# yuxiaoxiangyong/Multilateral-Temporal-view-Pyramid-Transformer-for-Video-Inpainting-Detection

Measured on AMD Instinct MI355X. Metric: clips/sec fwd (B=8,T=5,224x224), higher is better.
Workload: dtype f32; 1 GPU; full Mumpy forward (3 temporal views, pyramid decoder), B=8 clips/GPU, T=5, 224x224, fp32, tubelets (5,4,1); global_batch=8, launch=hipGraph replay, fork/join over HIP streams (independent branches co-scheduled), parallelism=batch-sharded x1, one metric all-reduce

## Files before the change

### multilateral-temporal-view-pyramid-transformer-for-video-inpainting-detection_amd/csrc/abi.cpp

```cpp
#include <stdarg.h>
#include <stdio.h>
#include <string.h>
#include "common.h"
#include "../../include/mumpy_hip_ext.h"
#include "../../include/mumpy_hip_ext2.h"
#include "../../include/mumpy_hip_ext3.h"
#include "../../include/mumpy_hip_ext4.h"
#include "../../include/mumpy_hip_ext5.h"
#include "../../include/mumpy_hip_ext6.h"
#include "../../include/mumpy_hip_ext7.h"
#include "../../include/mumpy_hip_ext8.h"
#include "../../include/mumpy_hip_ext9.h"
#include "../../include/mumpy_hip_ext10.h"
#include "../../include/mumpy_perturb.h"

namespace mumpy {
static thread_local char g_err[512] = "";
void set_error(const char* fmt, ...) {
    va_list ap;
    va_start(ap, fmt);
    vsnprintf(g_err, sizeof(g_err), fmt, ap);
    va_end(ap);
}
thread_local Route g_route;
static thread_local char g_route_text[160] = "";
static const char* format_route() {
    static const char* const addr[] = {"dense", "rows", "kseg", "conv"};
    static const char* const ln[] = {"none", "producer", "consumer"};
    static const char* const red[] = {"none", "one", "two-in-one", "taps"};
    const Route& r = g_route;
    char* t = g_route_text;
    const size_t n = sizeof(g_route_text);
    switch (r.family) {
    case Route::TILED: snprintf(t, n, "tiled tile=%d ks=%d np=%d addr=%s", r.tile, r.ks, r.np, addr[r.addr & 3]); break;
    case Route::TILED16: snprintf(t, n, "tiled16 tile=%d ks=%d np=%d addr=%s", r.tile, r.ks, r.np, addr[r.addr & 3]); break;
    case Route::WS:
        snprintf(t, n, "ws sched=%s P=%d ln=%s addr=%s", r.split ? "split" : "whole", r.passes, ln[r.ln < 3 ? r.ln : 0], addr[r.addr & 3]);
        break;
    case Route::WS64: snprintf(t, n, "ws64 P=%d addr=dense", r.passes); break;
    case Route::WS16: snprintf(t, n, "ws16 P=%d addr=dense", r.passes); break;
    case Route::XGEMM: {
        char dx[24] = "-", dw[24] = "-";
        if (r.prod[0].wt) snprintf(dx, sizeof(dx), "%dx%d", r.prod[0].wt, r.prod[0].ks);
        if (r.prod[1].wt) snprintf(dw, sizeof(dw), "%dx%d", r.prod[1].wt, r.prod[1].ks);
        snprintf(t, n, "xgemm np=%d addr=%s dx=%s dw=%s reduce=%s", r.np, addr[r.addr & 3], dx, dw, red[r.reduce & 3]);
        break;
    }
    default: snprintf(t, n, "none");
    }
    if (r.dual && r.family != Route::NONE) {
        const size_t len = strlen(t);
        snprintf(t + len, n - len, r.family == Route::XGEMM ? " gate=gelu" : " dual=z");
    }
    return t;
}
#ifdef MUMPY_TUNING
#include <stdlib.h>
int tune_int(const char* name, int dflt) {
    const char* v = getenv(name);
    return v ? atoi(v) : dflt;
}
const char* tune_str(const char* name) { return getenv(name); }
#endif
}

extern "C" int mumpy_tuning_build(void) {
#ifdef MUMPY_TUNING
    return 1;
#else
    return 0;
#endif
}

extern "C" int mumpy_abi_version(void) { return MUMPY_ABI_VERSION; }
extern "C" int mumpy_ext_version(void) { return MUMPY_EXT_VERSION; }
extern "C" int mumpy_ext2_version(void) { return MUMPY_EXT2_VERSION; }
extern "C" int mumpy_ext3_version(void) { return MUMPY_EXT3_VERSION; }
extern "C" int mumpy_ext4_version(void) { return MUMPY_EXT4_VERSION; }
extern "C" int mumpy_ext5_version(void) { return MUMPY_EXT5_VERSION; }
extern "C" int mumpy_ext6_version(void) { return MUMPY_EXT6_VERSION; }
extern "C" int mumpy_ext7_version(void) { return MUMPY_EXT7_VERSION; }
extern "C" int mumpy_ext8_version(void) { return MUMPY_EXT8_VERSION; }
extern "C" int mumpy_ext9_version(void) { return MUMPY_EXT9_VERSION; }
extern "C" int mumpy_ext10_version(void) { return MUMPY_EXT10_VERSION; }
extern "C" int mumpy_perturb_version(void) { return MUMPY_PERTURB_VERSION; }
extern "C" const char* mumpy_last_error(void) { return mumpy::g_err; }
extern "C" const char* mumpy_last_route(void) { return mumpy::format_route(); }
```

### multilateral-temporal-view-pyramid-transformer-for-video-inpainting-detection_amd/csrc/cva_fused.hip

```cpp
#include "cva_pairing.h"
#include "../../include/mumpy_hip_ext8.h"
using namespace mumpy;

namespace {

constexpr int BK = 32, LDR = 36;
constexpr int LDH = 20;

typedef __bf16 bf16x8 __attribute__((ext_vector_type(8)));
typedef __bf16 bf16x4 __attribute__((ext_vector_type(4)));

__device__ __forceinline__ void put_bf16x4(float* img, int dw, f32x4 v) {
    *reinterpret_cast<uint2*>(img + dw) = __builtin_bit_cast(uint2, __builtin_convertvector(v, bf16x4));
}
__device__ __forceinline__ bf16x8 frag_bf16(const float* row_h, int st) { return *reinterpret_cast<const bf16x8*>(row_h + 8 * st); }

__device__ __forceinline__ void divmod49(unsigned m, unsigned& q, unsigned& r) {
    q = (unsigned)(((uint64_t)m * 2804876602ull) >> 37);
    r = m - 49u * q;
}

template <int C, bool MM16, bool GROUPED>
__global__ __launch_bounds__(256, 2) void deform_sample_kv_kernel(const float* __restrict__ x2, const float* __restrict__ pos,
                                                                  const float* __restrict__ Wkv, const float* __restrict__ bkv,
                                                                  float* __restrict__ kv, int Hs2, int W, int nWx, int nW2,
                                                                  CvaPairing<GROUPED> pair, int M, unsigned gn) {
    constexpr int BM = 64, BN = 192, TN = 3, N = 2 * C, K = C, CG = C / 3, NK = K / BK, CPG = CG / BK;
    constexpr int A_LD = BM / 32, B_LD = BN / 32;
    __shared__ __attribute__((aligned(16))) float lds[2][(BM + BN) * (MM16 ? LDH : LDR)];
    const int tid = threadIdx.x, lane = tid & 63, wave = tid >> 6;
    const int c = lane & 31, h = lane >> 5, wm = wave >> 1, wn = wave & 1;
    const unsigned wgid = xcd_major_id(blockIdx.x, gridDim.x);
    const unsigned tm = wgid / gn, tn = wgid - tm * gn;
    const int m0 = (int)tm * BM, n0 = (int)tn * BN;
    const int ld_row = tid >> 3, ld_c4 = tid & 7;

    const float* abase[A_LD];
    const float* apos[A_LD];
    int aoff[A_LD][4];
    float aw[A_LD][4];
#pragma unroll
    for (int i = 0; i < A_LD; ++i) {
        int m = m0 + ld_row + 32 * i;
        if (m > M - 1) m = M - 1;
        unsigned b2, p;
        divmod49((unsigned)m, b2, p);
        const unsigned b = b2 / (unsigned)nW2, n = b2 - b * (unsigned)nW2;
        const unsigned wy = n / (unsigned)nWx, wx = n - wy * (unsigned)nWx;
        abase[i] = x2 + (((int64_t)b * Hs2 + wy * WS) * W + wx * WS) * C + 4 * ld_c4;
        apos[i] = pos + ((int64_t)cva_q_window(b2, pair) * 3 * WT + p) * 2;
    }
    auto set_group = [&](int g) {
#pragma unroll
        for (int i = 0; i < A_LD; ++i) {
            const float gy = apos[i][g * WT * 2], gx = apos[i][g * WT * 2 + 1];
            const float iy = ((gy + 1.0f) * 0.5f) * 6.0f;
            const float ix = ((gx + 1.0f) * 0.5f) * 6.0f;
            const float y0f = floorf(iy), x0f = floorf(ix);
            const int y0 = (int)y0f, x0 = (int)x0f;
            const float wgt[4] = {(x0f + 1.0f - ix) * (y0f + 1.0f - iy), (ix - x0f) * (y0f + 1.0f - iy),
                                  (x0f + 1.0f - ix) * (iy - y0f), (ix - x0f) * (iy - y0f)};
#pragma unroll
            for (int e = 0; e < 4; ++e) {
                const int yy = y0 + (e >> 1), xx = x0 + (e & 1);
                const bool ok = (unsigned)yy < (unsigned)WS && (unsigned)xx < (unsigned)WS;
                aw[i][e] = ok ? wgt[e] : 0.f;
                aoff[i][e] = ok ? (yy * W + xx) * C : 0;
            }
        }
    };
    const float* brow[B_LD];
#pragma unroll
    for (int i = 0; i < B_LD; ++i) {
        int n = n0 + ld_row + 32 * i;
        if (n > N - 1) n = N - 1;
        brow[i] = Wkv + (int64_t)n * K + 4 * ld_c4;
    }
    f32x4 areg[A_LD], breg[B_LD];
    auto gload = [&](int kc) {
        const int k0 = kc * BK;
#pragma unroll
        for (int i = 0; i < A_LD; ++i) {
            const float* s = abase[i] + k0;
            f32x4 r = *reinterpret_cast<const f32x4*>(s + aoff[i][0]) * aw[i][0];
            r += *reinterpret_cast<const f32x4*>(s + aoff[i][1]) * aw[i][1];
            r += *reinterpret_cast<const f32x4*>(s + aoff[i][2]) * aw[i][2];
            r += *reinterpret_cast<const f32x4*>(s + aoff[i][3]) * aw[i][3];
            areg[i] = r;
        }
#pragma unroll
        for (int i = 0; i < B_LD; ++i) breg[i] = *reinterpret_cast<const f32x4*>(brow[i] + k0);
    };
    auto lstore = [&](int buf) {
        if constexpr (MM16) {
#pragma unroll
            for (int i = 0; i < A_LD; ++i) put_bf16x4(lds[buf], (ld_row + 32 * i) * LDH + 2 * ld_c4, areg[i]);
#pragma unroll
            for (int i = 0; i < B_LD; ++i) put_bf16x4(lds[buf], (BM + ld_row + 32 * i) * LDH + 2 * ld_c4, breg[i]);
        } else {
#pragma unroll
            for (int i = 0; i < A_LD; ++i) *reinterpret_cast<f32x4*>(&lds[buf][(ld_row + 32 * i) * LDR + 4 * ld_c4]) = areg[i];
#pragma unroll
            for (int i = 0; i < B_LD; ++i) *reinterpret_cast<f32x4*>(&lds[buf][(BM + ld_row + 32 * i) * LDR + 4 * ld_c4]) = breg[i];
        }
    };
    f32x16 acc[TN];
#pragma unroll
    for (int j = 0; j < TN; ++j)
#pragma unroll
        for (int r = 0; r < 16; ++r) acc[j][r] = 0.f;
    auto compute = [&](int buf) {
        if constexpr (MM16) {
            const float* a_f = &lds[buf][(wm * 32 + c) * LDH + 4 * h];
            const float* b_f = &lds[buf][(BM + wn * 96 + c) * LDH + 4 * h];
#pragma unroll
            for (int st = 0; st < 2; ++st) {
                const bf16x8 fa = frag_bf16(a_f, st);
                bf16x8 fb[TN];
#pragma unroll
                for (int j = 0; j < TN; ++j) fb[j] = frag_bf16(b_f + 32 * j * LDH, st);
#pragma unroll
                for (int j = 0; j < TN; ++j) acc[j] = __builtin_amdgcn_mfma_f32_32x32x16_bf16(fa, fb[j], acc[j], 0, 0, 0);
            }
        } else {
            const float* a_f = &lds[buf][(wm * 32 + c) * LDR + 16 * h];
            const float* b_f = &lds[buf][(BM + wn * 96 + c) * LDR + 16 * h];
#pragma unroll
            for (int q = 0; q < 4; ++q) {
                const f32x4 fa = *reinterpret_cast<const f32x4*>(a_f + 4 * q);
                f32x4 fb[TN];
#pragma unroll
                for (int j = 0; j < TN; ++j) fb[j] = *reinterpret_cast<const f32x4*>(b_f + 32 * j * LDR + 4 * q);
#pragma unroll
                for (int e = 0; e < 4; ++e)
#pragma unroll
                    for (int j = 0; j < TN; ++j) acc[j] = __builtin_amdgcn_mfma_f32_32x32x2f32(fa[e], fb[j][e], acc[j], 0, 0, 0);
            }
        }
    };
    set_group(0);
    gload(0);
    lstore(0);
    __syncthreads();
    for (int kc = 0; kc < NK; ++kc) {
        if (kc + 1 < NK) {
            if ((kc + 1) % CPG == 0) set_group((kc + 1) / CPG);
            gload(kc + 1);
        }
        compute(kc & 1);
        if (kc + 1 < NK) lstore((kc + 1) & 1);
        __syncthreads();
    }
#pragma unroll
    for (int j = 0; j < TN; ++j) {
        const int n = n0 + wn * 96 + 32 * j + c;
        if (n >= N) continue;
        const float bv = bkv[n];
#pragma unroll
        for (int r = 0; r < 16; ++r) {
            const int m = m0 + wm * 32 + (r & 3) + 8 * (r >> 2) + 4 * h;
            if (m < M) kv[(int64_t)m * N + n] = acc[j][r] + bv;
        }
    }
}

template <int C, bool MM16>
__global__ __launch_bounds__(256, 2) void deform_out_combine_kernel(const float* __restrict__ o, const float* __restrict__ Wout,
                                                                   const float* __restrict__ bout, const float* __restrict__ x1,
                                                                   float* __restrict__ out, int H, int W, int nWx, int nWf, int MO,
                                                                   unsigned gn) {
    constexpr int BM = 64, BN = 64, K = C, NK = K / BK;
    constexpr int A_LD = BM / 32, B_LD = BN / 32;
    __shared__ __attribute__((aligned(16))) float lds[2][(BM + BN) * (MM16 ? LDH : LDR)];
    const int tid = threadIdx.x, lane = tid & 63, wave = tid >> 6;
    const int c = lane & 31, h = lane >> 5, wm = wave >> 1, wn = wave & 1;
    const unsigned wgid = xcd_major_id(blockIdx.x, gridDim.x);
    const unsigned tn = wgid / gn, tm = wgid - tn * gn;
    const int c0 = (int)tm * BM, m0 = (int)tn * BN;
    const int ld_row = tid >> 3, ld_c4 = tid & 7;
    const float* arow[A_LD];
    const float* brow[B_LD];
#pragma unroll
    for (int i = 0; i < A_LD; ++i) {
        int cc = c0 + ld_row + 32 * i;
        if (cc > C - 1) cc = C - 1;
        arow[i] = Wout + (int64_t)cc * K + 4 * ld_c4;
    }
#pragma unroll
    for (int i = 0; i < B_LD; ++i) {
        int m = m0 + ld_row + 32 * i;
        if (m > MO - 1) m = MO - 1;
        brow[i] = o + (int64_t)m * K + 4 * ld_c4;
    }
    f32x4 areg[A_LD], breg[B_LD];
    auto gload = [&](int kc) {
#pragma unroll
        for (int i = 0; i < A_LD; ++i) areg[i] = *reinterpret_cast<const f32x4*>(arow[i] + kc * BK);
#pragma unroll
        for (int i = 0; i < B_LD; ++i) breg[i] = *reinterpret_cast<const f32x4*>(brow[i] + kc * BK);
    };
    auto lstore = [&](int buf) {
        if constexpr (MM16) {
#pragma unroll
            for (int i = 0; i < A_LD; ++i) put_bf16x4(lds[buf], (ld_row + 32 * i) * LDH + 2 * ld_c4, areg[i]);
#pragma unroll
            for (int i = 0; i < B_LD; ++i) put_bf16x4(lds[buf], (BM + ld_row + 32 * i) * LDH + 2 * ld_c4, breg[i]);
        } else {
#pragma unroll
            for (int i = 0; i < A_LD; ++i) *reinterpret_cast<f32x4*>(&lds[buf][(ld_row + 32 * i) * LDR + 4 * ld_c4]) = areg[i];
#pragma unroll
            for (int i = 0; i < B_LD; ++i) *reinterpret_cast<f32x4*>(&lds[buf][(BM + ld_row + 32 * i) * LDR + 4 * ld_c4]) = breg[i];
        }
    };
    f32x16 acc;
#pragma unroll
    for (int r = 0; r < 16; ++r) acc[r] = 0.f;
    auto compute = [&](int buf) {
        if constexpr (MM16) {
            const float* a_f = &lds[buf][(wm * 32 + c) * LDH + 4 * h];
            const float* b_f = &lds[buf][(BM + wn * 32 + c) * LDH + 4 * h];
#pragma unroll
            for (int st = 0; st < 2; ++st)
                acc = __builtin_amdgcn_mfma_f32_32x32x16_bf16(frag_bf16(a_f, st), frag_bf16(b_f, st), acc, 0, 0, 0);
        } else {
            const float* a_f = &lds[buf][(wm * 32 + c) * LDR + 16 * h];
            const float* b_f = &lds[buf][(BM + wn * 32 + c) * LDR + 16 * h];
#pragma unroll
            for (int q = 0; q < 4; ++q) {
                const f32x4 fa = *reinterpret_cast<const f32x4*>(a_f + 4 * q), fb = *reinterpret_cast<const f32x4*>(b_f + 4 * q);
#pragma unroll
                for (int e = 0; e < 4; ++e) acc = __builtin_amdgcn_mfma_f32_32x32x2f32(fa[e], fb[e], acc, 0, 0, 0);
            }
        }
    };
    gload(0);
    lstore(0);
    __syncthreads();
    for (int kc = 0; kc < NK; ++kc) {
        if (kc + 1 < NK) gload(kc + 1);
        compute(kc & 1);
        if (kc + 1 < NK) lstore((kc + 1) & 1);
        __syncthreads();
    }
    const int m = m0 + wn * 32 + c;
    if (m >= MO) return;
    unsigned bw, pp;
    divmod49((unsigned)m, bw, pp);
    const unsigned b = bw / (unsigned)nWf, n = bw - b * (unsigned)nWf;
    const int wy = (int)(n / (unsigned)nWx), wx = (int)(n - (n / (unsigned)nWx) * (unsigned)nWx);
    const int64_t img = (int64_t)b * H * W;
    const int64_t win_base = (img + (int64_t)n * WT) * C;
#pragma unroll
    for (int r = 0; r < 16; ++r) {
        const int cc = c0 + wm * 32 + (r & 3) + 8 * (r >> 2) + 4 * h;
        if (cc >= C) continue;
        const int f = cc * WT + (int)pp;
        const int po = f / C, co = f - po * C;
        const int tok = window_token(wy, wx, po, H, W, 0);
        out[win_base + f] = x1[win_base + f] + x1[(img + tok) * C + co] + (acc[r] + bout[cc]);
    }
}

}

template <bool MM16>
static int sample_kv_launch(const char* who, const float* x2, const float* pos, const float* Wkv, const float* bkv, float* kv, int B,
                            int Hs2, int W, int C, int nq, int groups, void* stream) {
    MUMPY_REQUIRE(x2 && pos && Wkv && bkv && kv, MUMPY_ENULL, "%s: null pointer", who);
    MUMPY_REQUIRE(aligned16(x2) && aligned16(Wkv) && aligned16(kv), MUMPY_EALIGN, "%s: pointers must be 16-byte aligned", who);
    MUMPY_REQUIRE(B > 0 && Hs2 > 0 && W > 0 && Hs2 % WS == 0 && W % WS == 0 && nq > 0, MUMPY_EINVAL,
                  "%s: bad grid (%d,%d) / nq=%d", who, Hs2, W, nq);
    MUMPY_REQUIRE(C == 96 || C == 192 || C == 384 || C == 768, MUMPY_EINVAL,
                  "%s: C=%d is not one of the encoder widths 96/192/384/768", who, C);
    const int nWx = W / WS, nW2 = (Hs2 / WS) * nWx;
    const int64_t nwin = (int64_t)B * nW2, M = nwin * WT;
    MUMPY_REQUIRE(M < (1ll << 31) - 64, MUMPY_ERANGE, "%s: too many windows", who);
    const unsigned gn = (unsigned)((2 * C + 191) / 192);
    const int64_t grid = ((M + 63) / 64) * gn;
    MUMPY_REQUIRE(grid < (1ll << 31), MUMPY_ERANGE, "%s: too many tiles", who);
    CvaPairing<true> pg;
    const int bad = cva_grouping(who, nwin, nq, B, groups, &pg);
    if (bad) return bad;
    const CvaPairing<false> p1 = {nq};
#define MUMPY_SKV_AS(C_, G_, P_)                                                                                             \
    hipLaunchKernelGGL((deform_sample_kv_kernel<C_, MM16, G_>), dim3((unsigned)grid), dim3(256), 0, as_stream(stream), x2, pos, Wkv, \
                       bkv, kv, Hs2, W, nWx, nW2, P_, (int)M, gn)
#define MUMPY_SKV(C_)                                                                                                        \
    if (groups > 1) MUMPY_SKV_AS(C_, true, pg); else MUMPY_SKV_AS(C_, false, p1)
    switch (C) {
        case 96: MUMPY_SKV(96); break;
        case 192: MUMPY_SKV(192); break;
        case 384: MUMPY_SKV(384); break;
        default: MUMPY_SKV(768); break;
    }
#undef MUMPY_SKV
#undef MUMPY_SKV_AS
    MUMPY_CHECK_LAUNCH(who);
    return 0;
}

template <bool MM16>
static int out_combine_launch(const char* who, const float* o, const float* Wout, const float* bout, const float* x1, float* out,
                              int B, int H, int W, int C, void* stream) {
    MUMPY_REQUIRE(o && Wout && bout && x1 && out, MUMPY_ENULL, "%s: null pointer", who);
    MUMPY_REQUIRE(x1 != out, MUMPY_EINVAL, "%s: out must not alias x1", who);
    MUMPY_REQUIRE(aligned16(o) && aligned16(Wout), MUMPY_EALIGN, "%s: pointers must be 16-byte aligned", who);
    MUMPY_REQUIRE(B > 0 && H > 0 && W > 0 && H % WS == 0 && W % WS == 0, MUMPY_EINVAL, "%s: bad grid (%d,%d)", who, H, W);
    MUMPY_REQUIRE(C == 96 || C == 192 || C == 384 || C == 768, MUMPY_EINVAL,
                  "%s: C=%d is not one of the encoder widths 96/192/384/768", who, C);
    const int nWx = W / WS, nWf = (H / WS) * nWx;
    const int64_t MO = (int64_t)B * nWf * WT;
    MUMPY_REQUIRE(MO * 49 < (1ll << 31) && MO < (1ll << 31) - 64, MUMPY_ERANGE, "%s: too many windows", who);
    const unsigned gn = (unsigned)((C + 63) / 64);
    const int64_t grid = ((MO + 63) / 64) * gn;
#define MUMPY_OC(C_)                                                                                                         \
    hipLaunchKernelGGL((deform_out_combine_kernel<C_, MM16>), dim3((unsigned)grid), dim3(256), 0, as_stream(stream), o, Wout, bout, \
                       x1, out, H, W, nWx, nWf, (int)MO, gn)
    switch (C) {
        case 96: MUMPY_OC(96); break;
        case 192: MUMPY_OC(192); break;
        case 384: MUMPY_OC(384); break;
        default: MUMPY_OC(768); break;
    }
#undef MUMPY_OC
    MUMPY_CHECK_LAUNCH(who);
    return 0;
}

extern "C" int mumpy_deform_sample_kv_fwd(const float* x2, const float* pos, const float* Wkv, const float* bkv, float* kv, int B,
                                          int Hs2, int W, int C, int nq, void* stream) {
    return sample_kv_launch<false>("deform_sample_kv", x2, pos, Wkv, bkv, kv, B, Hs2, W, C, nq, 1, stream);
}

extern "C" int mumpy_deform_sample_kv_grouped_fwd(const float* x2, const float* pos, const float* Wkv, const float* bkv, float* kv,
                                                  int B, int Hs2, int W, int C, int nq, int groups, void* stream) {
    return sample_kv_launch<false>("deform_sample_kv_grouped", x2, pos, Wkv, bkv, kv, B, Hs2, W, C, nq, groups, stream);
}

extern "C" int mumpy_deform_sample_kv_mm16_grouped_fwd(const float* x2, const float* pos, const float* Wkv, const float* bkv,
                                                       float* kv, int B, int Hs2, int W, int C, int nq, int groups, void* stream) {
    return sample_kv_launch<true>("deform_sample_kv_mm16_grouped", x2, pos, Wkv, bkv, kv, B, Hs2, W, C, nq, groups, stream);
}

extern "C" int mumpy_deform_sample_kv_mm16_fwd(const float* x2, const float* pos, const float* Wkv, const float* bkv, float* kv,
                                               int B, int Hs2, int W, int C, int nq, void* stream) {
    return sample_kv_launch<true>("deform_sample_kv_mm16", x2, pos, Wkv, bkv, kv, B, Hs2, W, C, nq, 1, stream);
}

extern "C" int mumpy_deform_out_combine_fwd(const float* o, const float* Wout, const float* bout, const float* x1, float* out, int B,
                                            int H, int W, int C, void* stream) {
    return out_combine_launch<false>("deform_out_combine", o, Wout, bout, x1, out, B, H, W, C, stream);
}

extern "C" int mumpy_deform_out_combine_mm16_fwd(const float* o, const float* Wout, const float* bout, const float* x1, float* out,
                                                 int B, int H, int W, int C, void* stream) {
    return out_combine_launch<true>("deform_out_combine_mm16", o, Wout, bout, x1, out, B, H, W, C, stream);
}
```

### multilateral-temporal-view-pyramid-transformer-for-video-inpainting-detection_amd/mumpy_hip/lib.py

```python
import ctypes
import os
import subprocess
from typing import NamedTuple

_HERE = os.path.dirname(os.path.abspath(__file__))
_PKG = os.path.dirname(_HERE)
_LIB = None

c_f = ctypes.c_void_p
c_i = ctypes.c_int
c_l = ctypes.c_int64
c_fl = ctypes.c_float
c_d = ctypes.c_double


class Surface(NamedTuple):
    header: str
    version_fn: str
    version: int
    signatures: dict


SURFACES = [
    Surface("mumpy_hip.h", "mumpy_abi_version", 2, {
        "mumpy_layernorm_fwd": [c_f, c_f, c_f, c_f, c_l, c_i, c_fl, c_f],
        "mumpy_layernorm_bf16_fwd": [c_f, c_f, c_f, c_f, c_l, c_i, c_fl, c_f],
        "mumpy_linear_fwd": [c_f, c_f, c_f, c_f, c_f, c_l, c_i, c_i, c_i, c_f],
        "mumpy_linear_bf16s_fwd": [c_f, c_f, c_f, c_f, c_f, c_l, c_i, c_i, c_i, c_i, c_f],
        "mumpy_window_attention_bf16_fwd": [c_f, c_f, c_f, c_f, c_f, c_i, c_i, c_i, c_i, c_i, c_i, c_fl, c_f],
        "mumpy_window_attention_bf16mm_fwd": [c_f, c_f, c_f, c_f, c_f, c_i, c_i, c_i, c_i, c_i, c_i, c_fl, c_f],
        "mumpy_linear_ws_fwd": [c_f, c_f, c_f, c_f, c_f, c_l, c_i, c_i, c_i, c_f, c_l, c_f],
        "mumpy_linear_wsz_fwd": [c_f, c_f, c_f, c_f, c_f, c_l, c_i, c_i, c_i, c_f, c_l, c_f],
        "mumpy_linear_rd_fwd": [c_f, c_f, c_f, c_f, c_f, c_l, c_i, c_i, c_i, c_f],
        "mumpy_window_attention_bg_fwd": [c_f, c_f, c_f, c_f, c_f, c_i, c_i, c_i, c_i, c_i, c_i, c_fl, c_f],
        "mumpy_linear_workspace_bytes": [c_l, c_i, c_i],
        "mumpy_tuning_build": [],
        "mumpy_workspace_status": [c_f, ctypes.POINTER(ctypes.c_int)],
        "mumpy_linear_ln_tiles": [c_l, c_i, c_i],
        "mumpy_linear_lnx_fwd": [c_f, c_f, c_f, c_f, c_f, c_l, c_i, c_i, c_i, c_f, c_l, c_f, c_f, c_i, c_f, c_fl, c_f],
        "mumpy_linear_rows_fwd": [c_f, c_l, c_l, c_f, c_f, c_f, c_f, c_l, c_i, c_i, c_i, c_f, c_l, c_f],
        "mumpy_linear_rows_kseg_fwd": [c_f, c_l, c_l, c_i, c_i, c_f, c_f, c_f, c_f, c_l, c_i, c_i, c_i, c_f, c_l, c_f],
        "mumpy_gn_stats_nhwc_fwd": [c_f, c_f, c_i, c_l, c_i, c_i, c_i, c_f],
        "mumpy_gn_apply_resample_nhwc_fwd": [c_f, c_f, c_i, c_f, c_f, c_i, c_fl, c_i, c_i, c_i, c_i, c_i, c_f, c_f, c_f, c_i, c_i,
                                             c_i, c_i, c_i, c_i, c_f],
        "mumpy_conv2d_nhwc_fwd": [c_f, c_f, c_f, c_f, c_f, c_i, c_i, c_i, c_i, c_i, c_i, c_i, c_i, c_f, c_l, c_f],
        "mumpy_conv2d_workspace_bytes": [c_i, c_i, c_i, c_i, c_i, c_i, c_i],
        "mumpy_avgpool2_pad_nhwc_fwd": [c_f, c_f, c_i, c_i, c_i, c_i, c_i, c_i, c_f],
        "mumpy_copy_rows_fwd": [c_f, c_l, c_f, c_l, c_l, c_i, c_f],
        "mumpy_merge_views_fwd": [c_f, c_f, c_f, c_f, c_i, c_i, c_i, c_i, c_i, c_i, c_i, c_i, c_i, c_f],
        "mumpy_trunk_head_fwd": [c_f, c_f, c_f, c_f, c_f, c_i, c_i, c_i, c_i, c_f],
        "mumpy_final_conv_fwd": [c_f, c_f, c_f, c_f, c_f, c_i, c_i, c_i, c_i, c_fl, c_f],
        "mumpy_window_attention_fwd": [c_f, c_f, c_f, c_f, c_f, c_i, c_i, c_i, c_i, c_i, c_i, c_fl, c_f],
        "mumpy_deform_offsets_fwd": [c_f, c_f, c_f, c_f, c_f, c_f, c_f, c_i, c_i, c_i, c_i, c_f],
        "mumpy_deform_sample_fwd": [c_f, c_f, c_f, c_i, c_i, c_i, c_i, c_i, c_f],
        "mumpy_deform_attention_fwd": [c_f, c_f, c_f, c_f, c_i, c_i, c_i, c_i, c_i, c_fl, c_f],
        "mumpy_deform_sample_kv_fwd": [c_f, c_f, c_f, c_f, c_f, c_i, c_i, c_i, c_i, c_i, c_f],
        "mumpy_deform_out_combine_fwd": [c_f, c_f, c_f, c_f, c_f, c_i, c_i, c_i, c_i, c_f],
        "mumpy_deform_attention_mm16_fwd": [c_f, c_f, c_f, c_f, c_i, c_i, c_i, c_i, c_i, c_fl, c_f],
        "mumpy_window_attention_plan": [c_i, c_i, c_i, c_i],
        "mumpy_window_attention_bf16_plan": [c_i, c_i, c_i, c_i],
        "mumpy_deform_attention_plan": [c_i, c_i, c_i, c_i, c_i],
        "mumpy_deform_sample_kv_mm16_fwd": [c_f, c_f, c_f, c_f, c_f, c_i, c_i, c_i, c_i, c_i, c_f],
        "mumpy_deform_out_combine_mm16_fwd": [c_f, c_f, c_f, c_f, c_f, c_i, c_i, c_i, c_i, c_f],
        "mumpy_deform_combine_fwd": [c_f, c_f, c_f, c_i, c_i, c_i, c_i, c_f],
        "mumpy_faf_fwd": [c_f, c_f, c_f, c_f, c_f, c_i, c_i, c_i, c_i, c_i, c_i, c_f],
        "mumpy_patch_embed_fwd": [c_f, c_f, c_f, c_f, c_f, c_f, c_i, c_i, c_i, c_i, c_i, c_i, c_fl, c_f],
        "mumpy_patch_merge_ln_fwd": [c_f, c_f, c_f, c_f, c_i, c_i, c_i, c_i, c_fl, c_f],
        "mumpy_temporal_attention_fwd": [c_f, c_f, c_l, c_i, c_i, c_i, c_fl, c_f],
        "mumpy_attention_probs_fwd": [c_f, c_f, c_f, c_l, c_i, c_i, c_i, c_i, c_l, c_l, c_l, c_l, c_l, c_fl, c_f],
        "mumpy_temporal_attention_q_fwd": [c_f, c_f, c_l, c_i, c_i, c_i, c_i, c_fl, c_f],
        "mumpy_sigmoid_threshold_fwd": [c_f, c_f, c_l, c_fl, c_f],
        "mumpy_add_fwd": [c_f, c_f, c_f, c_l, c_f],
        "mumpy_normalize_u8_fwd": [c_f, c_f, c_l, c_i, c_i, ctypes.POINTER(ctypes.c_float), ctypes.POINTER(ctypes.c_float), c_f],
        "mumpy_resize_nearest_table": [c_i, c_i, ctypes.POINTER(ctypes.c_int32)],
        "mumpy_resize_normalize_u8_fwd": [c_f, c_f, c_f, c_f, c_l, c_i, c_i, c_i, c_i, ctypes.POINTER(ctypes.c_float), ctypes.POINTER(ctypes.c_float), c_f],
        "mumpy_mask_loss_workspace_bytes": [c_i, c_l],
        "mumpy_mask_loss_fwd_bwd": [c_f, c_f, c_f, c_f, c_f, c_l, c_i, c_l, c_fl, c_fl, c_f],
        "mumpy_layernorm_bwd_workspace_bytes": [c_l, c_i],
        "mumpy_layernorm_bwd": [c_f, c_f, c_f, c_f, c_f, c_f, c_f, c_f, c_l, c_l, c_i, c_fl, c_i, c_f],
        "mumpy_gelu_fwd": [c_f, c_f, c_l, c_f],
        "mumpy_gelu_bwd": [c_f, c_f, c_f, c_l, c_f],
        "mumpy_transpose_fwd": [c_f, c_f, c_l, c_l, c_f],
        "mumpy_col_sum_workspace_bytes": [c_l, c_i],
        "mumpy_col_sum_fwd": [c_f, c_f, c_f, c_l, c_l, c_i, c_f],
        "mumpy_final_conv_bwd_workspace_bytes": [c_i, c_i, c_i],
        "mumpy_final_conv_bwd": [c_f, c_f, c_f, c_f, c_f, c_f, c_f, c_l, c_i, c_i, c_i, c_i, c_f],
        "mumpy_patch_gather_fwd": [c_f, c_f, c_l, c_i, c_i, c_i, c_i, c_f],
        "mumpy_conv_weight_dgrad_fwd": [c_f, c_f, c_i, c_i, c_i, c_i, c_f],
        "mumpy_conv2d_wgrad_workspace_bytes": [c_i, c_i, c_i, c_i, c_i, c_i, c_i],
        "mumpy_conv2d_wgrad_nhwc": [c_f, c_f, c_f, c_i, c_i, c_i, c_i, c_i, c_i, c_i, c_i, c_f, c_l, c_f],
        "mumpy_linear_bwd_workspace_bytes": [c_l, c_i, c_i],
        "mumpy_linear_bwd": [c_f, c_f, c_f, c_f, c_f, c_f, c_l, c_i, c_i, c_i, c_f, c_l, c_f],
        "mumpy_window_attention_bwd_workspace_bytes": [c_i, c_i, c_i, c_i],
        "mumpy_window_attention_bwd": [c_f, c_f, c_f, c_f, c_f, c_i, c_f, c_f, c_f, c_f, c_l, c_i, c_i, c_i, c_i, c_i, c_fl, c_i, c_f],
        "mumpy_window_attention_bwd_csr": [c_f, c_f, c_f, c_f, c_f, c_i, c_f, c_f, c_f, c_f, c_f, c_l, c_i, c_i, c_i, c_i, c_i, c_fl, c_i, c_f],
        "mumpy_window_attention_mm16_fwd": [c_f, c_f, c_f, c_f, c_f, c_i, c_i, c_i, c_i, c_i, c_i, c_fl, c_f],
        "mumpy_window_attention_mm16_bwd_workspace_bytes": [c_i, c_i, c_i, c_i],
        "mumpy_window_attention_mm16_bwd": [c_f, c_f, c_f, c_f, c_f, c_i, c_f, c_f, c_f, c_f, c_f, c_l, c_i, c_i, c_i, c_i, c_i, c_fl, c_i, c_f],
        "mumpy_relpos_bias_expand_fwd": [c_f, c_f, c_f, c_i, c_f],
        "mumpy_gn_bwd_workspace_bytes": [c_i, c_l, c_i],
        "mumpy_gn_bwd_nhwc": [c_f, c_f, c_i, c_f, c_f, c_f, c_f, c_f, c_f, c_f, c_l, c_i, c_l, c_i, c_i, c_fl, c_i, c_f],
        "mumpy_upsample_bwd_nhwc": [c_f, c_f, c_i, c_i, c_i, c_i, c_i, c_i, c_f],
        "mumpy_temporal_attention_bwd": [c_f, c_f, c_f, c_l, c_i, c_i, c_i, c_fl, c_f],
        "mumpy_scale_samples_fwd": [c_f, c_f, c_f, c_i, c_l, c_f],
        "mumpy_dwconv5_window_fwd": [c_f, c_f, c_f, c_f, c_l, c_i, c_f],
        "mumpy_dwconv5_window_bwd_workspace_bytes": [c_l, c_i],
        "mumpy_dwconv5_window_bwd": [c_f, c_f, c_f, c_f, c_f, c_f, c_f, c_l, c_l, c_i, c_f],
        "mumpy_deform_attention_bwd_workspace_bytes": [c_l, c_i],
        "mumpy_deform_attention_bwd": [c_f, c_f, c_f, c_f, c_f, c_f, c_l, c_l, c_i, c_i, c_fl, c_f],
        "mumpy_deform_sample_bwd": [c_f, c_f, c_f, c_f, c_f, c_l, c_i, c_i, c_f],
        "mumpy_adamw_hyper": [ctypes.POINTER(ctypes.c_float), c_d, c_d, c_d, c_d, c_d, c_i, c_d],
        "mumpy_adamw_step_dev": [c_f, c_f, c_f, c_f, c_l, c_f, c_f],
        "mumpy_adamw_step": [c_f, c_f, c_f, c_f, c_l, c_d, c_d, c_d, c_d, c_d, c_i, c_d, c_f],
        "mumpy_sgd_step": [c_f, c_f, c_f, c_l, c_d, c_d, c_d, c_d, c_i, c_d, c_f],
        "mumpy_sgd_hyper": [ctypes.POINTER(ctypes.c_float), c_d, c_d, c_d, c_d, c_i, c_d],
        "mumpy_sgd_step_dev": [c_f, c_f, c_f, c_l, c_f, c_i, c_f],
        "mumpy_rmsprop_step": [c_f, c_f, c_f, c_f, c_l, c_d, c_d, c_d, c_d, c_d, c_d, c_f],
        "mumpy_rmsprop_hyper": [ctypes.POINTER(ctypes.c_float), c_d, c_d, c_d, c_d, c_d, c_d],
        "mumpy_rmsprop_step_dev": [c_f, c_f, c_f, c_f, c_l, c_f, c_f],
        "mumpy_grad_norm_partials": [c_l],
        "mumpy_grad_norm_partial": [c_f, c_l, c_f, c_f],
        "mumpy_grad_norm_finish": [c_f, c_f, c_f, c_f, c_i, c_i, c_d, c_f, c_f],
    }),
    Surface("mumpy_hip_ext.h", "mumpy_ext_version", 1, {
        "mumpy_adamw_gate_hyper": [ctypes.POINTER(ctypes.c_double), c_d, c_d, c_d, c_i],
        "mumpy_update_gate": [c_f, c_i, c_f, c_f, c_f, c_i, c_f, c_f, c_f],
        "mumpy_adamw_step_gated_dev": [c_f, c_f, c_f, c_f, c_l, c_f, c_f, c_f],
        "mumpy_sgd_step_gated_dev": [c_f, c_f, c_f, c_l, c_f, c_i, c_f, c_f],
        "mumpy_rmsprop_step_gated_dev": [c_f, c_f, c_f, c_f, c_l, c_f, c_f, c_f],
    }),
    Surface("mumpy_hip_ext2.h", "mumpy_ext2_version", 2, {
        "mumpy_deform_attention_mm16_bwd_workspace_bytes": [c_l, c_i, c_i],
        "mumpy_deform_attention_mm16_bwd": [c_f, c_f, c_f, c_f, c_f, c_f, c_l, c_l, c_i, c_i, c_fl, c_f],
        "mumpy_linear_gelu_dual_fwd": [c_f, c_f, c_f, c_f, c_f, c_l, c_i, c_i, c_i, c_f, c_l, c_f],
        "mumpy_linear_gelu_bwd_workspace_bytes": [c_l, c_i, c_i],
        "mumpy_linear_gelu_bwd": [c_f, c_f, c_f, c_f, c_f, c_f, c_f, c_l, c_i, c_i, c_i, c_f, c_l, c_f],
    }),
    Surface("mumpy_hip_ext3.h", "mumpy_ext3_version", 1, {
        "mumpy_augment_stage_u8_fwd": [c_f, c_f, c_f, c_f, c_f, c_f, c_f, c_l, c_i, c_l, c_i, c_i, c_i, ctypes.POINTER(ctypes.c_float),
                                       ctypes.POINTER(ctypes.c_float), c_f],
    }),
    Surface("mumpy_hip_ext4.h", "mumpy_ext4_version", 1, {
        "mumpy_augment_warp_u8_fwd": [c_f, c_f, c_f, c_f, c_f, c_f, c_f, c_f, c_f, c_f, c_f, c_f, c_f, c_l, c_i, c_l, c_i, c_i, c_i,
                                      ctypes.POINTER(ctypes.c_float), ctypes.POINTER(ctypes.c_float), c_f],
    }),
    Surface("mumpy_hip_ext5.h", "mumpy_ext5_version", 1, {
        "mumpy_clip_window_u8_fwd": [c_f, c_f, c_f, c_f, c_f, c_l, c_i, c_l, c_i, c_i, c_i, c_i, ctypes.POINTER(ctypes.c_float),
                                     ctypes.POINTER(ctypes.c_float), c_f],
        "mumpy_mask_score_u8_fwd": [c_f, c_f, c_f, c_f, c_f, c_l, c_l, c_l, c_f],
        "mumpy_frame_metrics_fwd": [c_f, c_l, c_l, c_f, c_i, c_f],
    }),
    Surface("mumpy_hip_ext6.h", "mumpy_ext6_version", 1, {
        "mumpy_resize_bilinear_u8_fwd": [c_f, c_f, c_f, c_f, c_f, c_f, c_f, c_f, c_l, c_i, c_i, c_i, c_i, c_i, c_i, c_f],
    }),
    Surface("mumpy_hip_ext7.h", "mumpy_ext7_version", 1, {
        "mumpy_score_exceed_fwd": [c_f, c_f, c_f, c_f, c_f, c_l, c_l, c_l, c_i, c_f],
        "mumpy_sweep_metrics_fwd": [c_f, c_l, c_l, c_i, c_f, c_f, c_i, c_f],
    }),
    Surface("mumpy_hip_ext8.h", "mumpy_ext8_version", 1, {
        "mumpy_deform_sample_grouped_fwd": [c_f, c_f, c_f, c_i, c_i, c_i, c_i, c_i, c_i, c_f],
        "mumpy_deform_sample_kv_grouped_fwd": [c_f, c_f, c_f, c_f, c_f, c_i, c_i, c_i, c_i, c_i, c_i, c_f],
        "mumpy_deform_sample_kv_mm16_grouped_fwd": [c_f, c_f, c_f, c_f, c_f, c_i, c_i, c_i, c_i, c_i, c_i, c_f],
        "mumpy_deform_attention_grouped_fwd": [c_f, c_f, c_f, c_f, c_i, c_i, c_i, c_i, c_i, c_fl, c_i, c_f],
        "mumpy_deform_attention_mm16_grouped_fwd": [c_f, c_f, c_f, c_f, c_i, c_i, c_i, c_i, c_i, c_fl, c_i, c_f],
    }),
    Surface("mumpy_hip_ext9.h", "mumpy_ext9_version", 1, {
        "mumpy_deform_sample_grouped_bwd": [c_f, c_f, c_f, c_f, c_f, c_l, c_i, c_i, c_i, c_f],
        "mumpy_deform_attention_grouped_bwd": [c_f, c_f, c_f, c_f, c_f, c_f, c_l, c_l, c_i, c_i, c_fl, c_i, c_f],
        "mumpy_deform_attention_mm16_grouped_bwd": [c_f, c_f, c_f, c_f, c_f, c_f, c_l, c_l, c_i, c_i, c_fl, c_i, c_f],
    }),
    Surface("mumpy_hip_ext10.h", "mumpy_ext10_version", 1, {
        "mumpy_faf_bwd": [c_f, c_f, c_f, c_f, c_f, c_i, c_i, c_i, c_i, c_f],
        "mumpy_tokenize_dx": [c_f, c_f, c_f, c_f, c_f, c_i, c_i, c_i, c_i, c_i, c_i, c_i, c_i, c_i, c_i, c_i, c_f],
        "mumpy_pgd_step": [c_f, c_f, c_f, c_l, c_l, c_fl, ctypes.POINTER(ctypes.c_float), ctypes.POINTER(ctypes.c_float),
                           ctypes.POINTER(ctypes.c_float), c_f],
    }),
]
ABI_VERSION = SURFACES[0].version
SIGNATURES = {name: args for s in SURFACES for name, args in s.signatures.items()}

PERTURB = Surface("mumpy_perturb.h", "mumpy_perturb_version", 1, {
    "mumpy_jpeg_roundtrip_workspace_bytes": [c_l, c_i, c_i],
    "mumpy_jpeg_roundtrip_u8_fwd": [c_f, c_f, c_f, c_f, c_f, c_l, c_l, c_i, c_i, c_i, c_f],
    "mumpy_gaussian_blur_workspace_bytes": [c_l, c_i, c_i],
    "mumpy_gaussian_blur_u8_fwd": [c_f, c_f, c_f, c_f, c_l, c_l, c_i, c_i, c_f],
    "mumpy_resize_nearest_u8_fwd": [c_f, c_f, c_f, c_f, c_l, c_i, c_i, c_i, c_i, c_i, c_f],
})


def library_path() -> str:
    if "MUMPY_HIP_LIB" in os.environ:
        return os.environ["MUMPY_HIP_LIB"]
    name = "libmumpy_hip_tuning.so" if os.environ.get("MUMPY_TUNING", "0") == "1" else "libmumpy_hip.so"
    return os.path.join(_PKG, "lib", name)


def tuning_library_path() -> str:
    return os.path.join(_PKG, "lib", "libmumpy_hip_tuning.so")


def build_library(verbose: bool = False) -> str:
    r = subprocess.run(["make", "-C", os.path.join(_PKG, "csrc"), "-j8", "all", "tuning"], capture_output=True, text=True)
    if verbose or r.returncode:
        print(r.stdout[-4000:], r.stderr[-4000:])
    if r.returncode:
        raise RuntimeError("building libmumpy_hip.so failed (see output above)")
    return library_path()


def load_library():
    global _LIB
    if _LIB is not None:
        return _LIB
    path = library_path()
    if not os.path.exists(path):
        raise RuntimeError(
            f"libmumpy_hip.so not found at {path}: the HIP kernels are the only implementation of this package "
            "(no CPU/torch fallback). Build it with `python __graft_entry__.py` or `make -C <pkg>/csrc`.")
    lib = ctypes.CDLL(path)
    lib.mumpy_last_error.restype = ctypes.c_char_p
    lib.mumpy_last_route.restype = ctypes.c_char_p
    lib.mumpy_last_route.argtypes = []
    for s in SURFACES + [PERTURB]:
        version = getattr(lib, s.version_fn)
        version.restype, version.argtypes = c_i, []
        if version() != s.version:
            raise RuntimeError(f"{path}: {s.version_fn}() is {version()}, the binding of include/{s.header} expects {s.version}; rebuild")
        for name, args in s.signatures.items():
            fn = getattr(lib, name)
            fn.argtypes = args
            fn.restype = c_l if name.endswith("_bytes") else c_i
    _LIB = lib
    return lib
```

Before: 379.0 clips/s.

## Add shape-planned narrow-tile and deeper-prefetch variants for deformable CVA kernels

```diff
diff --git a/include/mumpy_cva_plan.h b/include/mumpy_cva_plan.h
--- /dev/null
+++ b/include/mumpy_cva_plan.h
@@ -0,0 +1,20 @@
+#ifndef MUMPY_CVA_PLAN_H
+#define MUMPY_CVA_PLAN_H
+
+#include "mumpy_hip.h"
+
+#ifdef __cplusplus
+extern "C" {
+#endif
+
+#define MUMPY_CVA_PLAN_VERSION 1
+int mumpy_cva_plan_version(void);
+
+int mumpy_deform_sample_kv_plan(int B, int Hs2, int W, int C);
+
+int mumpy_deform_out_combine_plan(int B, int H, int W, int C);
+
+#ifdef __cplusplus
+}
+#endif
+#endif
diff --git a/multilateral-temporal-view-pyramid-transformer-for-video-inpainting-detection_amd/csrc/abi.cpp b/multilateral-temporal-view-pyramid-transformer-for-video-inpainting-detection_amd/csrc/abi.cpp
--- a/multilateral-temporal-view-pyramid-transformer-for-video-inpainting-detection_amd/csrc/abi.cpp
+++ b/multilateral-temporal-view-pyramid-transformer-for-video-inpainting-detection_amd/csrc/abi.cpp
@@ -13,6 +13,7 @@
 #include "../../include/mumpy_hip_ext9.h"
 #include "../../include/mumpy_hip_ext10.h"
 #include "../../include/mumpy_perturb.h"
+#include "../../include/mumpy_cva_plan.h"
 
 namespace mumpy {
 static thread_local char g_err[512] = "";
@@ -84,5 +85,6 @@
 extern "C" int mumpy_ext9_version(void) { return MUMPY_EXT9_VERSION; }
 extern "C" int mumpy_ext10_version(void) { return MUMPY_EXT10_VERSION; }
 extern "C" int mumpy_perturb_version(void) { return MUMPY_PERTURB_VERSION; }
+extern "C" int mumpy_cva_plan_version(void) { return MUMPY_CVA_PLAN_VERSION; }
 extern "C" const char* mumpy_last_error(void) { return mumpy::g_err; }
 extern "C" const char* mumpy_last_route(void) { return mumpy::format_route(); }
diff --git a/multilateral-temporal-view-pyramid-transformer-for-video-inpainting-detection_amd/csrc/cva_fused.hip b/multilateral-temporal-view-pyramid-transformer-for-video-inpainting-detection_amd/csrc/cva_fused.hip
--- a/multilateral-temporal-view-pyramid-transformer-for-video-inpainting-detection_amd/csrc/cva_fused.hip
+++ b/multilateral-temporal-view-pyramid-transformer-for-video-inpainting-detection_amd/csrc/cva_fused.hip
@@ -1,5 +1,6 @@
 #include "cva_pairing.h"
 #include "../../include/mumpy_hip_ext8.h"
+#include "../../include/mumpy_cva_plan.h"
 using namespace mumpy;
 
 namespace {
@@ -20,12 +21,12 @@
     r = m - 49u * q;
 }
 
-template <int C, bool MM16, bool GROUPED>
+template <int C, bool MM16, bool GROUPED, int BN, int DEPTH>
 __global__ __launch_bounds__(256, 2) void deform_sample_kv_kernel(const float* __restrict__ x2, const float* __restrict__ pos,
                                                                   const float* __restrict__ Wkv, const float* __restrict__ bkv,
                                                                   float* __restrict__ kv, int Hs2, int W, int nWx, int nW2,
                                                                   CvaPairing<GROUPED> pair, int M, unsigned gn) {
-    constexpr int BM = 64, BN = 192, TN = 3, N = 2 * C, K = C, CG = C / 3, NK = K / BK, CPG = CG / BK;
+    constexpr int BM = 64, TN = BN / 64, N = 2 * C, K = C, CG = C / 3, NK = K / BK, CPG = CG / BK;
     constexpr int A_LD = BM / 32, B_LD = BN / 32;
     __shared__ __attribute__((aligned(16))) float lds[2][(BM + BN) * (MM16 ? LDH : LDR)];
     const int tid = threadIdx.x, lane = tid & 63, wave = tid >> 6;
@@ -76,32 +77,52 @@
         if (n > N - 1) n = N - 1;
         brow[i] = Wkv + (int64_t)n * K + 4 * ld_c4;
     }
-    f32x4 areg[A_LD], breg[B_LD];
-    auto gload = [&](int kc) {
+    f32x4 areg[DEPTH][A_LD], breg[DEPTH][B_LD];
+    f32x4 araw[DEPTH][A_LD][4];
+    float awt[DEPTH][A_LD][4];
+    auto gload = [&](int kc, int set) {
         const int k0 = kc * BK;
 #pragma unroll
         for (int i = 0; i < A_LD; ++i) {
             const float* s = abase[i] + k0;
+            if constexpr (DEPTH > 1) {
+#pragma unroll
+                for (int e = 0; e < 4; ++e) {
+                    araw[set][i][e] = *reinterpret_cast<const f32x4*>(s + aoff[i][e]);
+                    awt[set][i][e] = aw[i][e];
+                }
+                continue;
+            }
             f32x4 r = *reinterpret_cast<const f32x4*>(s + aoff[i][0]) * aw[i][0];
             r += *reinterpret_cast<const f32x4*>(s + aoff[i][1]) * aw[i][1];
             r += *reinterpret_cast<const f32x4*>(s + aoff[i][2]) * aw[i][2];
             r += *reinterpret_cast<const f32x4*>(s + aoff[i][3]) * aw[i][3];
-            areg[i] = r;
-        }
-#pragma unroll
-        for (int i = 0; i < B_LD; ++i) breg[i] = *reinterpret_cast<const f32x4*>(brow[i] + k0);
-    };
-    auto lstore = [&](int buf) {
+            areg[set][i] = r;
+        }
+#pragma unroll
+        for (int i = 0; i < B_LD; ++i) breg[set][i] = *reinterpret_cast<const f32x4*>(brow[i] + k0);
+    };
+    auto finish = [&](int set) {
+#pragma unroll
+        for (int i = 0; i < A_LD; ++i) {
+            f32x4 r = araw[set][i][0] * awt[set][i][0];
+            r += araw[set][i][1] * awt[set][i][1];
+            r += araw[set][i][2] * awt[set][i][2];
+            r += araw[set][i][3] * awt[set][i][3];
+            areg[set][i] = r;
+        }
+    };
+    auto lstore = [&](int buf, int set) {
         if constexpr (MM16) {
 #pragma unroll
-            for (int i = 0; i < A_LD; ++i) put_bf16x4(lds[buf], (ld_row + 32 * i) * LDH + 2 * ld_c4, areg[i]);
-#pragma unroll
-            for (int i = 0; i < B_LD; ++i) put_bf16x4(lds[buf], (BM + ld_row + 32 * i) * LDH + 2 * ld_c4, breg[i]);
+            for (int i = 0; i < A_LD; ++i) put_bf16x4(lds[buf], (ld_row + 32 * i) * LDH + 2 * ld_c4, areg[set][i]);
+#pragma unroll
+            for (int i = 0; i < B_LD; ++i) put_bf16x4(lds[buf], (BM + ld_row + 32 * i) * LDH + 2 * ld_c4, breg[set][i]);
         } else {
 #pragma unroll
-            for (int i = 0; i < A_LD; ++i) *reinterpret_cast<f32x4*>(&lds[buf][(ld_row + 32 * i) * LDR + 4 * ld_c4]) = areg[i];
-#pragma unroll
-            for (int i = 0; i < B_LD; ++i) *reinterpret_cast<f32x4*>(&lds[buf][(BM + ld_row + 32 * i) * LDR + 4 * ld_c4]) = breg[i];
+            for (int i = 0; i < A_LD; ++i) *reinterpret_cast<f32x4*>(&lds[buf][(ld_row + 32 * i) * LDR + 4 * ld_c4]) = areg[set][i];
+#pragma unroll
+            for (int i = 0; i < B_LD; ++i) *reinterpret_cast<f32x4*>(&lds[buf][(BM + ld_row + 32 * i) * LDR + 4 * ld_c4]) = breg[set][i];
         }
     };
     f32x16 acc[TN];
@@ -112,7 +133,7 @@
     auto compute = [&](int buf) {
         if constexpr (MM16) {
             const float* a_f = &lds[buf][(wm * 32 + c) * LDH + 4 * h];
-            const float* b_f = &lds[buf][(BM + wn * 96 + c) * LDH + 4 * h];
+            const float* b_f = &lds[buf][(BM + wn * 32 * TN + c) * LDH + 4 * h];
 #pragma unroll
             for (int st = 0; st < 2; ++st) {
                 const bf16x8 fa = frag_bf16(a_f, st);
@@ -124,7 +145,7 @@
             }
         } else {
             const float* a_f = &lds[buf][(wm * 32 + c) * LDR + 16 * h];
-            const float* b_f = &lds[buf][(BM + wn * 96 + c) * LDR + 16 * h];
+            const float* b_f = &lds[buf][(BM + wn * 32 * TN + c) * LDR + 16 * h];
 #pragma unroll
             for (int q = 0; q < 4; ++q) {
                 const f32x4 fa = *reinterpret_cast<const f32x4*>(a_f + 4 * q);
@@ -138,22 +159,49 @@
             }
         }
     };
-    set_group(0);
-    gload(0);
-    lstore(0);
-    __syncthreads();
-    for (int kc = 0; kc < NK; ++kc) {
-        if (kc + 1 < NK) {
-            if ((kc + 1) % CPG == 0) set_group((kc + 1) / CPG);
-            gload(kc + 1);
-        }
-        compute(kc & 1);
-        if (kc + 1 < NK) lstore((kc + 1) & 1);
+    if constexpr (DEPTH == 1) {
+        set_group(0);
+        gload(0, 0);
+        lstore(0, 0);
         __syncthreads();
+        for (int kc = 0; kc < NK; ++kc) {
+            if (kc + 1 < NK) {
+                if ((kc + 1) % CPG == 0) set_group((kc + 1) / CPG);
+                gload(kc + 1, 0);
+            }
+            compute(kc & 1);
+            if (kc + 1 < NK) lstore((kc + 1) & 1, 0);
+            __syncthreads();
+        }
+    } else {
+        auto stage = [&](int kc, int set) {
+            if (kc % CPG == 0) set_group(kc / CPG);
+            gload(kc, set);
+        };
+#pragma unroll
+        for (int d = 0; d < DEPTH; ++d)
+            if (d < NK) stage(d, d);
+        finish(0);
+        lstore(0, 0);
+        __syncthreads();
+        for (int kc0 = 0; kc0 < NK; kc0 += DEPTH) {
+#pragma unroll
+            for (int d = 0; d < DEPTH; ++d) {
+                const int kc = kc0 + d;
+                if (kc >= NK) break;
+                if (kc + DEPTH < NK) stage(kc + DEPTH, d);
+                compute(kc & 1);
+                if (kc + 1 < NK) {
+                    finish((d + 1) % DEPTH);
+                    lstore((kc + 1) & 1, (d + 1) % DEPTH);
+                }
+                __syncthreads();
+            }
+        }
     }
 #pragma unroll
     for (int j = 0; j < TN; ++j) {
-        const int n = n0 + wn * 96 + 32 * j + c;
+        const int n = n0 + wn * 32 * TN + 32 * j + c;
         if (n >= N) continue;
         const float bv = bkv[n];
 #pragma unroll
@@ -164,7 +212,7 @@
     }
 }
 
-template <int C, bool MM16>
+template <int C, bool MM16, int DEPTH>
 __global__ __launch_bounds__(256, 2) void deform_out_combine_kernel(const float* __restrict__ o, const float* __restrict__ Wout,
                                                                    const float* __restrict__ bout, const float* __restrict__ x1,
                                                                    float* __restrict__ out, int H, int W, int nWx, int nWf, int MO,
@@ -192,24 +240,24 @@
         if (m > MO - 1) m = MO - 1;
         brow[i] = o + (int64_t)m * K + 4 * ld_c4;
     }
-    f32x4 areg[A_LD], breg[B_LD];
-    auto gload = [&](int kc) {
-#pragma unroll
-        for (int i = 0; i < A_LD; ++i) areg[i] = *reinterpret_cast<const f32x4*>(arow[i] + kc * BK);
-#pragma unroll
-        for (int i = 0; i < B_LD; ++i) breg[i] = *reinterpret_cast<const f32x4*>(brow[i] + kc * BK);
-    };
-    auto lstore = [&](int buf) {
+    f32x4 areg[DEPTH][A_LD], breg[DEPTH][B_LD];
+    auto gload = [&](int kc, int set) {
+#pragma unroll
+        for (int i = 0; i < A_LD; ++i) areg[set][i] = *reinterpret_cast<const f32x4*>(arow[i] + kc * BK);
+#pragma unroll
+        for (int i = 0; i < B_LD; ++i) breg[set][i] = *reinterpret_cast<const f32x4*>(brow[i] + kc * BK);
+    };
+    auto lstore = [&](int buf, int set) {
         if constexpr (MM16) {
 #pragma unroll
-            for (int i = 0; i < A_LD; ++i) put_bf16x4(lds[buf], (ld_row + 32 * i) * LDH + 2 * ld_c4, areg[i]);
-#pragma unroll
-            for (int i = 0; i < B_LD; ++i) put_bf16x4(lds[buf], (BM + ld_row + 32 * i) * LDH + 2 * ld_c4, breg[i]);
+            for (int i = 0; i < A_LD; ++i) put_bf16x4(lds[buf], (ld_row + 32 * i) * LDH + 2 * ld_c4, areg[set][i]);
+#pragma unroll
+            for (int i = 0; i < B_LD; ++i) put_bf16x4(lds[buf], (BM + ld_row + 32 * i) * LDH + 2 * ld_c4, breg[set][i]);
         } else {
 #pragma unroll
-            for (int i = 0; i < A_LD; ++i) *reinterpret_cast<f32x4*>(&lds[buf][(ld_row + 32 * i) * LDR + 4 * ld_c4]) = areg[i];
-#pragma unroll
-            for (int i = 0; i < B_LD; ++i) *reinterpret_cast<f32x4*>(&lds[buf][(BM + ld_row + 32 * i) * LDR + 4 * ld_c4]) = breg[i];
+            for (int i = 0; i < A_LD; ++i) *reinterpret_cast<f32x4*>(&lds[buf][(ld_row + 32 * i) * LDR + 4 * ld_c4]) = areg[set][i];
+#pragma unroll
+            for (int i = 0; i < B_LD; ++i) *reinterpret_cast<f32x4*>(&lds[buf][(BM + ld_row + 32 * i) * LDR + 4 * ld_c4]) = breg[set][i];
         }
     };
     f32x16 acc;
@@ -233,14 +281,33 @@
             }
         }
     };
-    gload(0);
-    lstore(0);
-    __syncthreads();
-    for (int kc = 0; kc < NK; ++kc) {
-        if (kc + 1 < NK) gload(kc + 1);
-        compute(kc & 1);
-        if (kc + 1 < NK) lstore((kc + 1) & 1);
+    if constexpr (DEPTH == 1) {
+        gload(0, 0);
+        lstore(0, 0);
         __syncthreads();
+        for (int kc = 0; kc < NK; ++kc) {
+            if (kc + 1 < NK) gload(kc + 1, 0);
+            compute(kc & 1);
+            if (kc + 1 < NK) lstore((kc + 1) & 1, 0);
+            __syncthreads();
+        }
+    } else {
+#pragma unroll
+        for (int d = 0; d < DEPTH; ++d)
+            if (d < NK) gload(d, d);
+        lstore(0, 0);
+        __syncthreads();
+        for (int kc0 = 0; kc0 < NK; kc0 += DEPTH) {
+#pragma unroll
+            for (int d = 0; d < DEPTH; ++d) {
+                const int kc = kc0 + d;
+                if (kc >= NK) break;
+                if (kc + DEPTH < NK) gload(kc + DEPTH, d);
+                compute(kc & 1);
+                if (kc + 1 < NK) lstore((kc + 1) & 1, (d + 1) % DEPTH);
+                __syncthreads();
+            }
+        }
     }
     const int m = m0 + wn * 32 + c;
     if (m >= MO) return;
@@ -261,6 +328,50 @@
     }
 }
 
+}
+
+constexpr int SKV_NARROW_TILES = 256, SKV_DEEP_TILES = 85, OC_DEEP_TILES = 256;
+static int64_t sample_kv_tiles(int64_t M, int C) { return ((M + 63) / 64) * ((2 * C + 191) / 192); }
+static int64_t out_combine_tiles(int64_t MO, int C) { return ((MO + 63) / 64) * ((C + 63) / 64); }
+static int sample_kv_plan(int64_t M, int C) {
+    const int forced = tune_int("MUMPY_SKV_FORM", -1);
+    if (forced >= 0) return forced == 3 ? 3 : (forced & 1);
+    const int64_t tiles = sample_kv_tiles(M, C);
+    return tiles <= SKV_DEEP_TILES ? 3 : tiles <= SKV_NARROW_TILES ? 1 : 0;
+}
+static int out_combine_plan(int64_t MO, int C) {
+    const int forced = tune_int("MUMPY_OC_FORM", -1);
+    if (forced >= 0) return forced & 2;
+    return out_combine_tiles(MO, C) <= OC_DEEP_TILES ? 2 : 0;
+}
+
+extern "C" int mumpy_deform_sample_kv_plan(int B, int Hs2, int W, int C) {
+    MUMPY_REQUIRE(B > 0 && Hs2 > 0 && W > 0 && Hs2 % WS == 0 && W % WS == 0 && (C == 96 || C == 192 || C == 384 || C == 768), MUMPY_EINVAL,
+                  "deform_sample_kv_plan: bad shape (%d,%d,%d,%d)", B, Hs2, W, C);
+    return sample_kv_plan((int64_t)B * (Hs2 / WS) * (W / WS) * WT, C);
+}
+
+extern "C" int mumpy_deform_out_combine_plan(int B, int H, int W, int C) {
+    MUMPY_REQUIRE(B > 0 && H > 0 && W > 0 && H % WS == 0 && W % WS == 0 && (C == 96 || C == 192 || C == 384 || C == 768), MUMPY_EINVAL,
+                  "deform_out_combine_plan: bad shape (%d,%d,%d,%d)", B, H, W, C);
+    return out_combine_plan((int64_t)B * (H / WS) * (W / WS) * WT, C);
+}
+
+template <bool MM16, bool GROUPED, int BN, int DEPTH>
+static void sample_kv_go(int C, int64_t mtiles, void* stream, const float* x2, const float* pos, const float* Wkv, const float* bkv,
+                         float* kv, int Hs2, int W, int nWx, int nW2, CvaPairing<GROUPED> pair, int M) {
+    const unsigned gn = (unsigned)((2 * C + BN - 1) / BN);
+    const unsigned grid = (unsigned)(mtiles * gn);
+#define MUMPY_SKV(C_)                                                                                                                 \
+    hipLaunchKernelGGL((deform_sample_kv_kernel<C_, MM16, GROUPED, BN, DEPTH>), dim3(grid), dim3(256), 0, as_stream(stream), x2, pos, \
+                       Wkv, bkv, kv, Hs2, W, nWx, nW2, pair, M, gn)
+    switch (C) {
+        case 96: MUMPY_SKV(96); break;
+        case 192: MUMPY_SKV(192); break;
+        case 384: MUMPY_SKV(384); break;
+        default: MUMPY_SKV(768); break;
+    }
+#undef MUMPY_SKV
 }
 
 template <bool MM16>
@@ -275,28 +386,47 @@
     const int nWx = W / WS, nW2 = (Hs2 / WS) * nWx;
     const int64_t nwin = (int64_t)B * nW2, M = nwin * WT;
     MUMPY_REQUIRE(M < (1ll << 31) - 64, MUMPY_ERANGE, "%s: too many windows", who);
-    const unsigned gn = (unsigned)((2 * C + 191) / 192);
-    const int64_t grid = ((M + 63) / 64) * gn;
-    MUMPY_REQUIRE(grid < (1ll << 31), MUMPY_ERANGE, "%s: too many tiles", who);
+    const int form = MM16 ? 0 : sample_kv_plan(M, C);
+    const int64_t mtiles = (M + 63) / 64;
+    MUMPY_REQUIRE(mtiles * ((2 * C + 63) / 64) < (1ll << 31), MUMPY_ERANGE, "%s: too many tiles", who);
     CvaPairing<true> pg;
     const int bad = cva_grouping(who, nwin, nq, B, groups, &pg);
     if (bad) return bad;
     const CvaPairing<false> p1 = {nq};
-#define MUMPY_SKV_AS(C_, G_, P_)                                                                                             \
-    hipLaunchKernelGGL((deform_sample_kv_kernel<C_, MM16, G_>), dim3((unsigned)grid), dim3(256), 0, as_stream(stream), x2, pos, Wkv, \
-                       bkv, kv, Hs2, W, nWx, nW2, P_, (int)M, gn)
-#define MUMPY_SKV(C_)                                                                                                        \
-    if (groups > 1) MUMPY_SKV_AS(C_, true, pg); else MUMPY_SKV_AS(C_, false, p1)
-    switch (C) {
-        case 96: MUMPY_SKV(96); break;
-        case 192: MUMPY_SKV(192); break;
-        case 384: MUMPY_SKV(384); break;
-        default: MUMPY_SKV(768); break;
-    }
-#undef MUMPY_SKV
+#define MUMPY_SKV_AS(G_, P_, BN_, D_) \
+    sample_kv_go<MM16, G_, BN_, D_>(C, mtiles, stream, x2, pos, Wkv, bkv, kv, Hs2, W, nWx, nW2, P_, (int)M)
+#define MUMPY_SKV_FORM(BN_, D_)                                                                                              \
+    do {                                                                                                                     \
+        if (groups > 1) MUMPY_SKV_AS(true, pg, BN_, D_); else MUMPY_SKV_AS(false, p1, BN_, D_);                             \
+    } while (0)
+    if constexpr (MM16) {
+        MUMPY_SKV_FORM(192, 1);
+    } else {
+        switch (form) {
+            case 1: MUMPY_SKV_FORM(64, 1); break;
+            case 3: MUMPY_SKV_FORM(64, 2); break;
+            default: MUMPY_SKV_FORM(192, 1); break;
+        }
+    }
+#undef MUMPY_SKV_FORM
 #undef MUMPY_SKV_AS
     MUMPY_CHECK_LAUNCH(who);
     return 0;
+}
+
+template <bool MM16, int DEPTH>
+static void out_combine_go(int C, unsigned grid, void* stream, const float* o, const float* Wout, const float* bout, const float* x1,
+                           float* out, int H, int W, int nWx, int nWf, int MO, unsigned gn) {
+#define MUMPY_OC(C_)                                                                                                                \
+    hipLaunchKernelGGL((deform_out_combine_kernel<C_, MM16, DEPTH>), dim3(grid), dim3(256), 0, as_stream(stream), o, Wout, bout, x1, \
+                       out, H, W, nWx, nWf, MO, gn)
+    switch (C) {
+        case 96: MUMPY_OC(96); break;
+        case 192: MUMPY_OC(192); break;
+        case 384: MUMPY_OC(384); break;
+        default: MUMPY_OC(768); break;
+    }
+#undef MUMPY_OC
 }
 
 template <bool MM16>
@@ -312,17 +442,17 @@
     const int64_t MO = (int64_t)B * nWf * WT;
     MUMPY_REQUIRE(MO * 49 < (1ll << 31) && MO < (1ll << 31) - 64, MUMPY_ERANGE, "%s: too many windows", who);
     const unsigned gn = (unsigned)((C + 63) / 64);
-    const int64_t grid = ((MO + 63) / 64) * gn;
-#define MUMPY_OC(C_)                                                                                                         \
-    hipLaunchKernelGGL((deform_out_combine_kernel<C_, MM16>), dim3((unsigned)grid), dim3(256), 0, as_stream(stream), o, Wout, bout, \
-                       x1, out, H, W, nWx, nWf, (int)MO, gn)
-    switch (C) {
-        case 96: MUMPY_OC(96); break;
-        case 192: MUMPY_OC(192); break;
-        case 384: MUMPY_OC(384); break;
-        default: MUMPY_OC(768); break;
-    }
-#undef MUMPY_OC
+    const unsigned grid = (unsigned)(((MO + 63) / 64) * gn);
+#define MUMPY_OC_FORM(D_) out_combine_go<MM16, D_>(C, grid, stream, o, Wout, bout, x1, out, H, W, nWx, nWf, (int)MO, gn)
+    if constexpr (MM16) {
+        MUMPY_OC_FORM(1);
+    } else {
+        switch (out_combine_plan(MO, C)) {
+            case 2: MUMPY_OC_FORM(2); break;
+            default: MUMPY_OC_FORM(1); break;
+        }
+    }
+#undef MUMPY_OC_FORM
     MUMPY_CHECK_LAUNCH(who);
     return 0;
 }
diff --git a/multilateral-temporal-view-pyramid-transformer-for-video-inpainting-detection_amd/mumpy_hip/lib.py b/multilateral-temporal-view-pyramid-transformer-for-video-inpainting-detection_amd/mumpy_hip/lib.py
--- a/multilateral-temporal-view-pyramid-transformer-for-video-inpainting-detection_amd/mumpy_hip/lib.py
+++ b/multilateral-temporal-view-pyramid-transformer-for-video-inpainting-detection_amd/mumpy_hip/lib.py
@@ -187,6 +187,11 @@
     "mumpy_resize_nearest_u8_fwd": [c_f, c_f, c_f, c_f, c_l, c_i, c_i, c_i, c_i, c_i, c_f],
 })
 
+CVA_PLAN = Surface("mumpy_cva_plan.h", "mumpy_cva_plan_version", 1, {
+    "mumpy_deform_sample_kv_plan": [c_i, c_i, c_i, c_i],
+    "mumpy_deform_out_combine_plan": [c_i, c_i, c_i, c_i],
+})
+
 
 def library_path() -> str:
     if "MUMPY_HIP_LIB" in os.environ:
@@ -221,7 +226,7 @@
     lib.mumpy_last_error.restype = ctypes.c_char_p
     lib.mumpy_last_route.restype = ctypes.c_char_p
     lib.mumpy_last_route.argtypes = []
-    for s in SURFACES + [PERTURB]:
+    for s in SURFACES + [PERTURB, CVA_PLAN]:
         version = getattr(lib, s.version_fn)
         version.restype, version.argtypes = c_i, []
         if version() != s.version:
```

New measurement: 379.5 clips/s (median of 2 runs). About the same (+0.1%).
